# fulcrumgenomics/fgumi

Hardware: AMD Instinct MI355X
Metric: simplex consensus throughput, input raw reads/s (depth-8 x 150bp) (higher is better)
Workload: dtype f64

## Files before the change

fgumi_amd/csrc/api.cpp:

```cpp
#include <chrono>
#include <cstdio>
#include <stdexcept>
#include <cstring>
#include <mutex>
#include <map>
#include <mutex>
#include <string>
#include <thread>
#include "engine.h"
#include <gnu/libc-version.h>
#include <cmath>
#include "fastpath.h"
#include "host_common.h"
#include "simgen.h"
#include "canon_core.h"
#include "reject_core.h"
#include "aln_tags_core.h"

namespace fgx {
uint32_t launch_canon_molecules(hipStream_t s, bool codec, const canon::Params& P, const canon::CodecParams& PC, const uint8_t* d_blob,
                                const uint64_t* d_rec_off, const uint32_t* d_rec_len, const uint32_t* d_grp_first, const uint32_t* d_def, uint32_t nd,
                                const uint64_t* d_first, uint8_t* d_out, const uint64_t* d_out_off, uint32_t* d_out_len, int* d_status,
                                canon::Delta* d_delta, DevBuf& slabs);
void canon_layout_device(hipStream_t s, const uint32_t* d_rec_len, const uint32_t* d_grp_first, const uint32_t* d_def, uint32_t nd, unsigned long long* work,
// ... 1272 lines not shown
  double run = 0.0;
  for (uint32_t i = 0; i < n; i++) { run += (double)weights[i]; acc[i] = run; }
  const double total = acc[n - 1];
  for (uint32_t k = 1; k < world; k++) {
    const double want = total * (double)k / (double)world;
    const uint32_t idx = (uint32_t)(std::lower_bound(acc.begin(), acc.end(), want) - acc.begin());
    uint32_t c = idx + 1 > n ? n : idx + 1;
    if (c < cuts[k - 1]) c = cuts[k - 1];
    cuts[k] = c;
  }
  cuts[world] = n;
  for (uint32_t k = 1; k <= world; k++) if (cuts[k] < cuts[k - 1]) cuts[k] = cuts[k - 1];
  return 0;
}
uint32_t fgx_debug_last_split_chunks(const fgx_caller* c) { return (c && c->fast) ? c->fast->fp.last_split_chunks : 0u; }
uint32_t fgx_debug_last_big_families(const fgx_caller* c) { return (c && c->fast) ? c->fast->fp.last_big_families : 0u; }
uint32_t fgx_debug_last_meth_device(const fgx_caller* c) { return (c && c->fast) ? c->fast->fp.last_meth_device : 0u; }
uint32_t fgx_debug_last_deep_families(const fgx_caller* c) { return (c && c->fast) ? c->fast->fp.last_deep_families : 0u; }
void fgx_debug_last_split_builds(const fgx_caller* c, uint64_t* out4) {
  if (!out4) return;
  out4[0] = out4[1] = out4[2] = out4[3] = 0;
  if (c && c->fast) { const FastPath& f = c->fast->fp; out4[0] = f.last_packed_families; out4[1] = f.last_classic_families; out4[2] = f.last_split_build; out4[3] = f.last_first_stage_retries; }
}
void fgx_debug_last_chain(const fgx_caller* c, uint32_t* out2) { if (out2) { out2[0] = (c && c->fast) ? c->fast->fp.last_launches : 0u; out2[1] = (c && c->fast) ? c->fast->fp.last_host_syncs : 0u; } }
uint32_t fgx_debug_last_routed(const fgx_caller* c) { return (c && c->fast) ? c->fast->fp.last_routed : 0u; }
int fgx_debug_last_direct(const fgx_caller* c) { return (c && c->fast) ? c->fast->fp.last_direct : 0; }
void fgx_set_general_only(fgx_caller* c, int on) { if (c) c->general_only = on != 0; }
void fgx_set_fast_lds_bytes(fgx_caller* c, uint32_t bytes) { if (c) { if (!c->fast) c->fast = new FastState(); c->fast->fp.lds_tile_bytes_large = bytes; } }

int fgx_call_columns(fgx_caller* c, const uint8_t* bases, const uint8_t* quals, uint32_t n_cols, uint32_t depth, uint8_t* out_base,
                     uint8_t* out_qual, uint32_t* out_depth, uint32_t* out_errors) {
  if (!c) return 1;
  c->err.clear();
  try {
    ColumnBatch& B = c->batch;
    B.clear();
    std::vector<uint8_t> rb, rq;
    for (uint32_t j0 = 0; j0 < n_cols; j0 += 4096) {
      uint32_t w = std::min<uint32_t>(4096, n_cols - j0);
      uint32_t rd0 = (uint32_t)B.reads.size();
      for (uint32_t i = 0; i < depth; i++) {
        rb.resize(w); rq.resize(w);
        for (uint32_t k = 0; k < w; k++) { rb[k] = bases[(size_t)(j0 + k) * depth + i]; rq[k] = quals[(size_t)(j0 + k) * depth + i]; }
        B.add_read(rb.data(), rq.data(), w);
      }
      if (depth == 0) { B.add_job(rd0, 0, w); continue; }
// ... 129 lines not shown
```

fgumi_amd/csrc/fastpath.h:

```cpp
#pragma once
#include "engine.h"

namespace fgx {

constexpr int FAST_RX_CAP = 48;

struct EndDesc {
  uint64_t col_off;
  uint64_t first_off;
  uint64_t kept_off;
  uint32_t cons_len;
  uint32_t rec_size;
  uint16_t mi_off, cb_off;
  uint8_t mi_len, cb_len, rx_len, type;
  uint8_t has_cb, has_rx, valid, meth;
  char rx[FAST_RX_CAP];
};
struct MethSlot { uint32_t std_size, n_ml, mm_len, _pad; };

struct DuplexDesc {
  uint64_t a_off, b_off;
  uint32_t len;
  uint32_t first_rec;
  uint32_t cb_rec;
// ... 156 lines not shown
  const uint64_t* d_out_off;
  const uint64_t* d_slot_size;
  uint32_t n_slots;
  double ms_kernels, ms_k_family, ms_k_emit; uint64_t cols_used; uint64_t full_items;
};

struct FastPath {
  DevBuf d_ends, d_sizes, d_offsets, d_code, d_qual, d_depth, d_err, d_misc, d_deferred, d_out, d_scan_tmp, d_strings;
  uint32_t lds_tile_bytes = 12288;
  uint32_t lds_tile_bytes_large = 65536;
  DevBuf d_retry, d_bound, d_colbase, d_statslots, d_full_items, d_full_count, d_obs, d_retry2, d_retry_old;
  DevBuf d_w2img;
  DevBuf d_famdesc;
  DevBuf d_fwimg;
  DevBuf d_split_rec, d_split_fam, d_split_out, d_route, d_s2img;
  DevBuf d_big;
  uint32_t last_big_families = 0;
  uint32_t last_deep_families = 0;
  DevBuf d_deep_sizes, d_deep_row0, d_deep_rows, d_deep_fams, d_deep_out, d_deep_out2;
  DevBuf d_mflag, d_mu, d_mt, d_mslot, d_mcontigs;
  uint32_t last_meth_device = 0;
  uint32_t last_routed = 0;
  uint64_t last_packed_families = 0, last_classic_families = 0;
  uint32_t last_split_build = 0;
  uint32_t last_first_stage_retries = 0;
  uint32_t last_launches = 0, last_host_syncs = 0;
  DevBuf d_dir_size, d_dir_off, d_dir_base, d_slot_desc, d_slot_err, d_out2, d_scan_tmp2;
  bool direct_off = false;
  uint64_t dir_cap_min = 0;
  uint32_t dir_chunks_run = 0;
  int last_direct = 0;
  uint32_t lds_wave_bytes = 6144;
  uint32_t lds_wave_bytes_duplex = 8704;
  uint32_t lds_wave_bytes_codec = 5120;
  hipEvent_t ev[4] = {nullptr, nullptr, nullptr, nullptr};
  uint32_t pool_slack = 256; bool pool_init = false;
  uint32_t pool_div = 8;
  static constexpr int RUN_AGAIN_LARGER_POOL = -77;
  bool lds_attr_set = false, s2_attr_set = false, v2_attr_set = false;
  static constexpr int MAX_CHUNKS = 65;
  uint32_t last_split_chunks = 0;
  hipStream_t s2 = nullptr;
  hipEvent_t ev_chunk[MAX_CHUNKS] = {}, ev_cols[MAX_CHUNKS] = {}, ev_fin = nullptr, ev_sample = nullptr;
  int run(fgx_caller* c, const uint8_t* d_blob, uint64_t blob_len, const uint64_t* d_rec_off, const uint32_t* d_rec_len, uint32_t n_rec,
          const uint32_t* d_grp_first, uint32_t n_grp, FastResult* res);
  void release();
// ... 4 lines not shown
```

fgumi_amd/csrc/fastpath.hip:

```cpp
#if !defined(FGX_WAVEMU)
#include <hipcub/hipcub.hpp>
#endif
#include "bamrec.h"
#include "engine.h"
#include <cstdlib>
#include <memory>
#include <string>
#include <type_traits>
#include "fastpath.h"
#include "gate_core.h"
#include "packed_core.h"

#if defined(FGX_WAVEMU)
#define FGX_DYN_LDS(name) uint8_t* const name = wavemu::dyn_lds()
#define FGX_PIN(...) ((void)0)
#define FGX_UNDEF4(a, b, c, d) do { a = 0; b = 0; c = 0; d = 0; } while (0)
#define FGX_MEM_PIN() ((void)0)
#define FGX_CONST_AS
#else
#define FGX_DYN_LDS(name) extern __shared__ __align__(16) uint8_t name[]
#define FGX_PIN(...) asm volatile("" : __VA_ARGS__)
#define FGX_UNDEF4(a, b, c, d) asm volatile("" : "=v"(a), "=v"(b), "=v"(c), "=v"(d))
#define FGX_MEM_PIN() asm volatile("" ::: "memory")
#define FGX_CONST_AS __attribute__((address_space(4)))
// ... 3751 lines not shown
    hip_check(hipcub::DeviceScan::ExclusiveSum(fp.d_scan_tmp.p, tb, in, out, (int)n, s), what);
  }
  template <class Image> const void* table_image(DevBuf& d, void (*build)(Image&, const ConsensusTables&), const char* what) {
    if (!d.p) {
      const auto img = std::make_unique<Image>();
      build(*img, c->h_tables.t);
      d.reserve(sizeof(Image));
      hip_check(hipMemcpyAsync(d.p, img.get(), sizeof(Image), hipMemcpyHostToDevice, s), what);
      sync();
    }
    return d.p;
  }
  FastParams stage_params(uint32_t bytes, bool retry) {
    hip_check(hipMemsetAsync(cnt(MISC_N_RETRY), 0, 4, s), "memset");
    FastParams PS = P;
    PS.group_list = cur_list; PS.lds_wave_bytes = bytes;
    PS.retry = retry ? lists[out_list] : nullptr; PS.n_retry = cnt(MISC_N_RETRY);
    return PS;
  }
  void next_list(uint32_t n) { cur_list = lists[out_list]; n_cur = n; out_list ^= 1; }

  void set_up() {
    fp.last_meth_device = 0; fp.last_direct = 0; fp.last_split_chunks = 0;
    fp.last_routed = 0; fp.last_big_families = 0; fp.last_deep_families = 0; fp.last_packed_families = 0; fp.last_classic_families = 0; fp.last_split_build = 0; fp.last_first_stage_retries = 0;
    fp.d_ends.reserve((size_t)n_slots * (duplex ? sizeof(DuplexDesc) : codec ? sizeof(CodecDesc) : sizeof(EndDesc)));
    fp.d_sizes.reserve(((size_t)n_slots + 1) * 8);
    fp.d_offsets.reserve(((size_t)n_slots + 1) * 8);
    fp.d_deferred.reserve((size_t)n_grp * 4);
    fp.d_misc.reserve(MISC_WORDS * 8);
    hip_check(hipMemsetAsync(fp.d_misc.p, 0, MISC_WORDS * 8, s), "memset");
    misc = fp.d_misc.as<unsigned long long>();
    const std::string strs = c->prefix + c->rg;
    fp.d_strings.reserve(strs.size() + 16);
    if (!strs.empty()) hip_check(hipMemcpyAsync(fp.d_strings.p, strs.data(), strs.size(), hipMemcpyHostToDevice, s), "H2D strings");
    for (int i = 0; i < 4; i++) if (!fp.ev[i]) hip_check(hipEventCreate(&fp.ev[i]), "hipEventCreate");
    fp.d_bound.reserve(((size_t)n_grp + 1) * 8); fp.d_colbase.reserve(((size_t)n_grp + 1) * 8);
    fp.d_statslots.reserve((size_t)STAT_SLOTS * 32 * 8);
    hip_check(hipMemsetAsync(fp.d_statslots.p, 0, (size_t)STAT_SLOTS * 32 * 8, s), "memset");
    fp.d_famdesc.reserve((size_t)n_grp * 16);
    hip_check(hipEventRecord(c->ev0, s), "event");
    hip_check(hipEventRecord(fp.ev[0], s), "event");
    fpw = mean_recs >= 1.0 ? (uint32_t)(64.0 / mean_recs) : 16u;
    fpw = fpw < 1u ? 1u : fpw > 16u ? 16u : fpw;
    if (sw.split_fpw) fpw = sw.split_fpw;
    n_chunks = ps.chunks >= 1 ? (uint32_t)ps.chunks : std::min<uint32_t>(8u, std::max<uint32_t>(1u, n_grp / 150000u));
    if (n_chunks > (uint32_t)FastPath::MAX_CHUNKS - 1) n_chunks = FastPath::MAX_CHUNKS - 1;
    chunk_fam_raw = (n_grp + n_chunks - 1) / n_chunks;
// ... 502 lines not shown
    };
    read_counters();
    if ((duplex || codec) && (uint32_t)h_misc[MISC_N_SLOW] != 0) {
      if (codec) FGX_LAUNCH(k_emit_codec, wave_per_slot, dim3(256), 0, s, CE);
      else if (meth_dup) FGX_LAUNCH(HIP_KERNEL_NAME(k_emit_duplex<1>), wave_per_slot, dim3(256), 0, s, DE);
      else FGX_LAUNCH(HIP_KERNEL_NAME(k_emit_duplex<0>), wave_per_slot, dim3(256), 0, s, DE);
      read_counters();
    }
    float ms = 0, msf = 0, mse = 0;
    hip_check(hipEventElapsedTime(&ms, c->ev0, c->ev1), "elapsed");
    hip_check(hipEventElapsedTime(&msf, fp.ev[0], fp.ev[1]), "elapsed");
    hip_check(hipEventElapsedTime(&mse, fp.ev[2], fp.ev[3]), "elapsed");
    res->d_out = out_ptr;
    res->out_len = out_len;
    res->count = h_misc[MISC_STATS + 1];
    for (int i = 0; i < FGX_STATS_LEN; i++) res->stats[i] = h_misc[MISC_STATS + i];
    res->n_deferred = (uint32_t)(h_misc[MISC_N_DEFERRED] & 0xFFFFFFFFull);
    res->d_deferred = fp.d_deferred.as<uint32_t>();
    res->d_out_off = fp.d_offsets.as<uint64_t>();
    res->d_slot_size = fp.d_sizes.as<uint64_t>();
    res->n_slots = n_slots;
    res->ms_kernels = ms; res->ms_k_family = msf; res->ms_k_emit = mse;
    fp.last_packed_families = h_misc[MISC_BUILD_FAMILIES]; fp.last_classic_families = h_misc[MISC_BUILD_FAMILIES + 1];
    res->cols_used = h_misc[MISC_COLS_USED];
    res->full_items = n_full;
  }
};

int run_once(FastPath& fp, fgx_caller* c, const uint8_t* d_blob, uint64_t blob_len, const uint64_t* d_rec_off, const uint32_t* d_rec_len, uint32_t n_rec,
             const uint32_t* d_grp_first, uint32_t n_grp, FastResult* res) {
  memset(res, 0, sizeof(*res));
  fp.last_launches = 0; fp.last_host_syncs = 0;
  if (n_grp == 0) return 0;
  static const ProcessSwitches ps{};
  Batch b{fp, c, d_blob, blob_len, d_rec_off, d_rec_len, n_rec, d_grp_first, n_grp, res, ps};
  b.set_up();
  b.parse_first_chunk_early();
  b.bound_columns();
  b.fill_params();
  if (b.use_split) b.split_pipeline();
  if (b.simplex_v2) b.wave2_chain();
  b.family_wave_stages();
  b.deep_families();
  b.workgroup_families();
  if (const int rc = b.call_full()) return rc;
  if (b.direct) if (const int rc = b.check_direct()) return rc;
  b.place_records();
  b.write_records();
  return 0;
}

}

int FastPath::run(fgx_caller* c, const uint8_t* d_blob, uint64_t blob_len, const uint64_t* d_rec_off, const uint32_t* d_rec_len,
                  uint32_t n_rec, const uint32_t* d_grp_first, uint32_t n_grp, FastResult* res) {
  if (!pool_init) {
    if (const char* e = getenv("FGX_POOL_DIV")) { const long v = atol(e); if (v >= 1 && v <= (1 << 20)) pool_div = (uint32_t)v; }
    if (const char* e = getenv("FGX_POOL_SLACK")) { const long v = atol(e); if (v >= 1 && v <= 4096) pool_slack = (uint32_t)v; }
    pool_init = true;
  }
  for (;;) {
    const int rc = run_once(*this, c, d_blob, blob_len, d_rec_off, d_rec_len, n_rec, d_grp_first, n_grp, res);
    if (rc != RUN_AGAIN_LARGER_POOL) {
      if (const char* e = fgx_knob("FGX_S2_DEBUG")) if (atoi(e)) {
        uint32_t h[64];
        if (hipDeviceSynchronize() == hipSuccess && hipMemcpyFromSymbol(h, HIP_SYMBOL(g_s2_dbg), sizeof(h)) == hipSuccess) {
          fprintf(stderr, "[s2 packed] runs tried %u finished %u (columns for k_call_full %u) no room %u shape refused %u", h[0], h[1], h[2], h[3], h[42]);
          fprintf(stderr, "\n");
        }
      }
      return rc;
    }
  }
}

}

#if FGX_PHASE_TIMING
extern "C" int fgx_debug_phase_cycles(unsigned long long* out16, int reset) {
  unsigned long long h[64 * 16];
  if (hipMemcpyFromSymbol(h, HIP_SYMBOL(fgx::g_phase), sizeof(h)) != hipSuccess) return 1;
  for (int i = 0; i < 16; i++) { out16[i] = 0; for (int b = 0; b < 64; b++) out16[i] += h[b * 16 + i]; }
  if (reset) { memset(h, 0, sizeof(h)); if (hipMemcpyToSymbol(HIP_SYMBOL(fgx::g_phase), h, sizeof(h)) != hipSuccess) return 1; }
  return 0;
}
#endif
```

fgumi_amd/csrc/packed_core.h:

```cpp
#pragma once
#include <cstdint>
#include "consensus_math.h"

namespace fgx {
namespace pk {

constexpr uint32_t H = 0x80808080u;

FGX_HD uint32_t perm(uint32_t a, uint32_t b, uint32_t sel) {
#if defined(__HIP_DEVICE_COMPILE__)
  return __builtin_amdgcn_perm(a, b, sel);
#else
  const unsigned long long src = ((unsigned long long)a << 32) | b;
  uint32_t r = 0;
  for (int i = 0; i < 4; i++) {
    const uint32_t s = (sel >> (8 * i)) & 0xFFu;
    const uint32_t byte = s < 8u ? (uint32_t)(src >> (8 * s)) & 0xFFu : 0u;
    r |= byte << (8 * i);
  }
  return r;
#endif
}
FGX_HD uint32_t bitrev32(uint32_t x) {
#if defined(__HIP_DEVICE_COMPILE__)
// ... 79 lines not shown
    column_call(t, acc.s, acc.obs, &bi, &ql);
    if (bi == 0) t1[q] = ql;
  }
}

constexpr uint32_t T2_DIM = 94, T2_BYTES = T2_DIM * T2_DIM;
inline void fill_t2(uint8_t* t2 , const ConsensusTables& t) {
  for (uint32_t q1 = 0; q1 < T2_DIM; q1++)
    for (uint32_t q2 = 0; q2 < T2_DIM; q2++) {
      uint8_t& out = t2[q1 * T2_DIM + q2];
      out = 0xFF;
      ColumnAcc acc;
      acc.reset();
      acc.add(0, t.correct[q1], t.error_per_alt[q1]);
      acc.add(0, t.correct[q2], t.error_per_alt[q2]);
      if (!m_isfinite(acc.s[0]) || !m_isfinite(acc.s[1])) continue;
      int bi = -1;
      uint8_t ql = 0;
      column_call(t, acc.s, acc.obs, &bi, &ql);
      if (bi == 0) out = ql;
    }
}

}
}
```

fgumi_amd/csrc/simplex_split.inc:

```

#ifndef FGX_S2_OCC
#define FGX_S2_OCC 6
#endif
#ifndef FGX_S2_OCC_PACKED
#define FGX_S2_OCC_PACKED 7
#endif
#ifndef FGX_S2_PAIRS
#define FGX_S2_PAIRS 256
#endif

#ifndef FGX_S2_F32
#define FGX_S2_F32 1
#endif
#ifndef FGX_S2_FMASEL
#define FGX_S2_FMASEL 1
#endif
#ifndef FGX_S2_NOSUM
#define FGX_S2_NOSUM 1
#endif
#ifndef FGX_S2_PREGATE
#define FGX_S2_PREGATE 1
#endif
struct S2Lds {
  GateTables g;
// ... 468 lines not shown
__global__ __launch_bounds__(128) void k_split_parse(FastParams P, uint32_t g_begin, uint32_t n_grp, uint32_t fpw, uint64_t* __restrict__ bound, uint32_t max_ends,
                                                     uint4* __restrict__ fam_desc) {
  __shared__ __align__(16) uint8_t sTagCls[256];
  __shared__ __align__(16) uint8_t sWin[2 * SP_WAVE_LDS];
  fill_tag_classes(sTagCls);
  __syncthreads();
  const uint32_t wave = uni((blockIdx.x * blockDim.x + threadIdx.x) >> 6);
  const unsigned long long g0l = (unsigned long long)g_begin + (unsigned long long)wave * fpw;
  if (g0l >= n_grp) return;
  const uint32_t g0 = (uint32_t)g0l;
  const uint32_t nf = uni(n_grp - g0 < fpw ? n_grp - g0 : fpw);
  s2_parse_wave(P, g0, nf, sWin + (threadIdx.x >> 6) * SP_WAVE_LDS, sTagCls, bound, max_ends, fam_desc, [](uint32_t, uint32_t) {});
}

#if FGX_S2_PAIRS >= 256
#define S2_PAIR_OFF(q) ((q) << 4)
#else
#define S2_PAIR_OFF(q) (((q) < 93u ? (q) : 93u) << 4)
#endif
#ifndef FGX_S2_ABLATE
#define FGX_S2_ABLATE 0
#endif
#define S2_ABLATE_AFTER(k, sink) if (FGX_S2_ABLATE == (k)) { P.rec_sizes[slot0 + (lane & 1)] = (uint64_t)(sink); return; }
#ifndef FGX_S2_MIN_ITEMS
#define FGX_S2_MIN_ITEMS 8
#endif

#if FGX_S2_F32 && FGX_S2_FMASEL
#define S2_OBSERVE(q_, sb_, pr_) do { \
    const uint32_t w_q = (q_), w_c = ((uint32_t)(sb_) >> ish) & 15u; \
    const unsigned long long qm = __builtin_amdgcn_uicmp(w_q, min_bq, 35 ); \
    const unsigned long long bm = __builtin_amdgcn_uicmp(__builtin_amdgcn_ubfe(allow, w_c, 1u), 0u, 33 ); \
    suspect |= qm & ~bm; \
    const bool w_hit = __builtin_amdgcn_inverse_ballot_w64(qm & bm); \
    allow = w_hit ? 1u << w_c : allow; \
    const float w_sel = w_hit ? 1.0f : 0.0f; \
    const s2_f32x2 w_sel2 = {w_sel, w_sel}; \
    acc2 = __builtin_elementwise_fma((pr_), w_sel2, acc2);    \
    cntf += w_sel; \
  } while (0)
#else
#define S2_OBSERVE(q_, sb_, pr_) do { \
    const uint32_t w_q = (q_), w_c = ((uint32_t)(sb_) >> ish) & 15u; \
    const unsigned long long qm = __builtin_amdgcn_uicmp(w_q, min_bq, 35 ); \
    const unsigned long long bm = __builtin_amdgcn_uicmp(__builtin_amdgcn_ubfe(allow, w_c, 1u), 0u, 33 ); \
    suspect |= qm & ~bm; \
// ... 110 lines not shown
    if constexpr (TINY) {
      if (threadIdx.x < 24u) ((uint32_t*)&sL.t1[0])[threadIdx.x] = tiny_w;
      else if (threadIdx.x == 24u) sL.g.cap = tiny_w;
    } else {
      u32x4* const img_dst = (u32x4*)&sL;
#pragma unroll
      for (int u = 0; u < 6; u++) { const uint32_t ii = threadIdx.x + u * blockDim.x; if (ii < IMG_V) img_dst[ii] = im[u]; }
    }
  }
  const uint32_t body_off = d0.x, seq_rel = d0.y & 0xFFFF, l_seq = d0.y >> 16, clip = d0.z & 0xFFFF, ov_off1 = d0.z >> 16;
  const uint32_t ov_off2 = d0.w & 0xFFFF, ov_cnt = d0.w >> 16;
  const uint32_t slot = d1.x & 0xFF, mate_slot = (d1.x >> 8) & 0xFF, bits = (d1.x >> 16) & 0xFF, cb_len = d1.x >> 24;
  const uint32_t cb_rel = d1.y & 0xFFFF, mi_rel = d1.y >> 16, mi_len = d1.z & 0xFF, rx_rel = d1.z >> 16;
  const uint32_t ty = bits & 3u;
  const bool rev = (bits & 4u) != 0, has_cb = (bits & 8u) != 0;
  const unsigned long long lo_off = uniform_u64((unsigned long long)fd.x | ((unsigned long long)fd.y << 32));
  const uint8_t* const fbase = P.blob + lo_off;
  const uint32_t S0 = n * QS;
  if (act) *(uint2*)(W + ibase + 8u * slot) = make_uint2(body_off + seq_rel, l_seq);
  if constexpr (FUSED) wave_sync(); else __syncthreads();
  if (bail) return;
  {
    const uint32_t cpr = qc + sc, total = n * cpr;
    for (uint32_t t0 = 0; t0 < total; t0 += 256) {
      u32x4 v[4];
      uint32_t dst[4];
      bool on[4];
#pragma unroll
      for (int u = 0; u < 4; u++) {
        const uint32_t t = t0 + 64u * u + lane;
        const bool in = t < total;
        const uint32_t tt = in ? t : 0u;
        const uint32_t row = s2_mul24(tt, inv_cpr) >> 24;
        const uint32_t ch = tt - s2_mul24(row, cpr);
        const uint2 e = *(const uint2*)(W + ibase + 8u * row);
        const bool isq = ch < qc;
        const uint32_t c = isq ? ch : ch - qc;
        const uint32_t sbytes = (e.y + 1u) >> 1;
        const uint32_t src = e.x + (isq ? sbytes : 0u) + 16u * c;
        dst[u] = (isq ? row * QS : S0 + row * SS) + 16u * c;
        on[u] = in;
        const bool need_ld = in && 16u * c < (isq ? e.y : sbytes);
        u32x4 x = {0, 0, 0, 0};
        if (need_ld) __builtin_memcpy(&x, fbase + src, 16);
        v[u] = x;
      }
#pragma unroll
      for (int u = 0; u < 4; u++) if (on[u]) *(u32x4*)(W + dst[u]) = v[u];
    }
  }
  wave_sync();
  PH(1)
  const uint32_t my_q = slot * QS, my_s = S0 + slot * SS;
  if (__any(act && W[my_q] == 0xFF)) { to_route(); return; }
  S2_ABLATE_AFTER(1, W[my_s])

  const uint32_t min_bq = uni((uint32_t)P.min_input_bq & 0xFFu);
  uint32_t ov_agree = 0, ov_dis = 0, ov_corr = 0;
  {
    auto shared_base = [&](const bool in, const uint32_t o1, const uint32_t o2, const uint32_t q1, const uint32_t q2, const uint32_t sh1, const uint32_t sh2) {
      const uint32_t c1 = ((uint32_t)W[o1] >> sh1) & 15, c2 = ((uint32_t)W[o2] >> sh2) & 15;
      const uint32_t qa = W[q1], qb = W[q2];
      const bool valid = in && (c1 > c2 ? c1 : c2) != 15;
      const bool agree = c1 == c2;
      const uint32_t sm = qa + qb, nq = sm < 93 ? sm : 93;
      const int32_t d = (int32_t)qa - (int32_t)qb;
      const uint32_t ad = (uint32_t)(d < 0 ? -d : d), dq = ad < FGX_MIN_PHRED ? (uint32_t)FGX_MIN_PHRED : ad;
      const uint32_t cb = d == 0 ? 15u : d > 0 ? c1 : c2;
      const uint32_t newq = agree ? nq : dq;
      const bool drop = newq < min_bq;
      const uint32_t x1 = drop ? c1 : agree ? 0u : (c1 ^ cb), x2 = drop ? c2 : agree ? 0u : (c2 ^ cb);
      const bool changed = nq != qa || nq != qb;
      if (valid) {
        atomicXor((uint32_t*)(W + (o1 & ~3u)), x1 << (8 * (o1 & 3) + sh1));
        atomicXor((uint32_t*)(W + (o2 & ~3u)), x2 << (8 * (o2 & 3) + sh2));
        W[q1] = (uint8_t)newq; W[q2] = (uint8_t)newq;
      }
      const uint32_t na = (uint32_t)__popcll(__ballot(valid && agree)), nd = (uint32_t)__popcll(__ballot(valid && !agree));
      ov_agree += na; ov_dis += nd;
      ov_corr += (uint32_t)__popcll(__ballot(valid && agree && changed)) + 2u * nd;
    };
    const unsigned long long om = __ballot(act && ov_cnt != 0);
    if (om) {
      const uint32_t np = (uint32_t)__popcll(om), fp = (uint32_t)__builtin_ctzll(om);
      const uint32_t cn0 = rlane(ov_cnt, fp);
      if (ov_uniform && np > 1u && cn0 < 64u) {
        const uint32_t oo1 = rlane(ov_off1, fp), oo2 = rlane(ov_off2, fp);
        if (act && ov_cnt != 0) *(uint16_t*)(W + ibase + 2u * (uint32_t)__popcll(om & below)) = (uint16_t)(slot | (mate_slot << 8));
        wave_sync();
        const uint32_t inv = uni((uint32_t)(1048576.0f / (float)cn0) + 2u);
        const uint32_t total = np * cn0;
        for (uint32_t t0 = 0; t0 < total; t0 += 64) {
          const uint32_t t = t0 + lane;
          const bool in = t < total;
          const uint32_t tt = in ? t : 0u;
          const uint32_t pk = s2_mul24(tt, inv) >> 20, w = tt - s2_mul24(pk, cn0);
          const uint32_t rows = *(const uint16_t*)(W + ibase + 2u * pk), r1 = rows & 0xFF, r2 = rows >> 8;
          const uint32_t i1 = oo1 + w, i2 = oo2 + w;
          shared_base(in, S0 + r1 * SS + (i1 >> 1), S0 + r2 * SS + (i2 >> 1), r1 * QS + i1, r2 * QS + i2, (~i1 & 1) << 2, (~i2 & 1) << 2);
        }
      } else {
        const uint32_t mt_q = mate_slot * QS, mt_s = S0 + mate_slot * SS;
        const uint32_t my_q0 = slot * QS, my_s0 = S0 + slot * SS;
        for (unsigned long long pm = om; pm; pm &= pm - 1) {
          const uint32_t a = (uint32_t)__builtin_ctzll(pm);
          const uint32_t sa = rlane(my_s0, a), qa0 = rlane(my_q0, a), sb = rlane(mt_s, a), qb0 = rlane(mt_q, a);
          const uint32_t cn = rlane(ov_cnt, a);
          const uint32_t i1 = rlane(ov_off1, a) + lane, i2 = rlane(ov_off2, a) + lane;
          uint32_t o1 = sa + (i1 >> 1), o2 = sb + (i2 >> 1), q1 = qa0 + i1, q2 = qb0 + i2;
          const uint32_t sh1 = (~i1 & 1) << 2, sh2 = (~i2 & 1) << 2;
          for (uint32_t w0 = 0; w0 < cn; w0 += 64, o1 += 32, o2 += 32, q1 += 64, q2 += 64) shared_base(w0 + lane < cn, o1, o2, q1, q2, sh1, sh2);
        }
      }
    }
  }
  const uint32_t ov_bases = ov_agree + ov_dis;
  wave_sync();
  PH(3)
  S2_ABLATE_AFTER(3, ov_bases + ov_corr + W[my_s])

  const uint32_t fl = l_seq > clip ? l_seq - clip : 0u;
  if (act) {
    uint32_t z0, z1;
    if (!rev) { z0 = fl; z1 = ty == 2u ? len_b : len_a; } else { z0 = 0; z1 = clip < l_seq ? clip : l_seq; }
// ... 343 lines not shown
  bool ires_asked = false;
  auto run_cols_packed = [&](const uint32_t cnt_a, const uint32_t cnt_b, const uint32_t m, const bool last_run) -> bool {
    const uint32_t nsafe = P.s2_nsafe;
    const uint32_t ga = cnt_a ? (len_a + 7u) >> 3 : 0u, gb = cnt_b ? (len_b + 7u) >> 3 : 0u;
    const bool dbg = (P.s2_packed & 2u) != 0;
    if (!(P.s2_packed && m >= nsafe && m <= S2_PACKED_MAX_ROWS && P.min_reads <= nsafe && min_bq <= 128u && ((QS & 7u) | (SS & 3u)) == 0u && ga + gb <= 64u &&
          S0 + s2_mul24(n, SS) < 65536u && lc_a + lc_b < 65536u)) {
      if (dbg && lane == 0) atomicAdd(&g_s2_dbg[42], 1u);
      return false;
    }
    if (dbg && lane == 0) atomicAdd(&g_s2_dbg[0], 1u);
    const bool in_b = lane >= ga, inl = lane < ga + gb;
    const uint32_t k = inl ? (in_b ? lane - ga : lane) : 0u;
    const bool lrev = (in_b ? rev_b : rev_a) != 0;
    const uint32_t lenE = in_b ? len_b : len_a, cntE = in_b ? cnt_b : cnt_a;
    const uint32_t rowE = in_b ? m_a : 0u;
    const uint32_t qaddr0 = s2_mul24(rowE, QS) + 8u * k, saddr0 = S0 + s2_mul24(rowE, SS) + 4u * k;
    const uint32_t H = pk::H;
    uint32_t nfl, nfh;
    pk::count_masks(lenE, k, &nfl, &nfh);
    const uint32_t mb4 = min_bq * 0x01010101u;
    pk::Acc A;
    pk::acc_reset(A);
    {
      uint32_t qj = qaddr0, sj = saddr0, j = 0;
      for (; j + 4 <= m; j += 4, qj += 4 * QS, sj += 4 * SS) {
        const uint2 q0 = *(const uint2*)(W + qj), q1 = *(const uint2*)(W + qj + QS), q2 = *(const uint2*)(W + qj + 2 * QS), q3 = *(const uint2*)(W + qj + 3 * QS);
        const uint32_t b0 = *(const uint32_t*)(W + sj), b1_ = *(const uint32_t*)(W + sj + SS), b2_ = *(const uint32_t*)(W + sj + 2 * SS), b3_ = *(const uint32_t*)(W + sj + 3 * SS);
        pk::acc_row(A, q0.x, q0.y, b0, mb4, nfl, nfh); pk::acc_row(A, q1.x, q1.y, b1_, mb4, nfl, nfh);
        pk::acc_row(A, q2.x, q2.y, b2_, mb4, nfl, nfh); pk::acc_row(A, q3.x, q3.y, b3_, mb4, nfl, nfh);
      }
      for (; j < m; j++, qj += QS, sj += SS) { const uint2 q0 = *(const uint2*)(W + qj); const uint32_t b0 = *(const uint32_t*)(W + sj); pk::acc_row(A, q0.x, q0.y, b0, mb4, nfl, nfh); }
    }
    PH(9)
    pk::Out F;
    pk::finalize(A, inl, lrev, lenE, cntE, k, nsafe, sT.cap, P.min_cons_bq, P.min_reads, F);
    const int32_t c_lo = F.c_lo, lo_s = F.lo_s, hi_s = F.hi_s;
    const uint32_t* const code2 = F.code2; const uint32_t* const qual2 = F.qual2; const uint32_t* const dep4 = F.dep4;
    const uint32_t* const flag2 = F.flag2; const uint32_t* const full2 = F.valid2;
    PH(10)
    uint32_t fm = (flag2[0] >> 7) | (flag2[1] >> 3);
    const uint32_t fc = (uint32_t)__builtin_popcount(fm);
    const unsigned long long pb0 = __ballot((fc & 1u) != 0), pb1 = __ballot((fc & 2u) != 0), pb2 = __ballot((fc & 4u) != 0), pb3 = __ballot((fc & 8u) != 0);
    const uint32_t T = uni((uint32_t)__popcll(pb0) + 2u * (uint32_t)__popcll(pb1) + 4u * (uint32_t)__popcll(pb2) + 8u * (uint32_t)__popcll(pb3));
    const uint32_t oc0 = (in_b ? offB : offA) + (uint32_t)c_lo;
    const uint32_t list = (P.lds_wave_bytes - 8u * T) & ~7u;
// ... 91 lines not shown
    } else {
      if (ne >= 1u && surv_a == 1u) single_end(mem_a, lc_a, offA);
      if (ne == 2u && surv_b == 1u) single_end(mem_b, lc_b, offB);
    }
    const bool both = multi_a && multi_b && m_a == m_b;
    const uint32_t nruns = both ? 1u : (multi_a ? 1u : 0u) + (multi_b ? 1u : 0u);
#pragma unroll 1
    for (uint32_t ri = 0; ri < nruns && !gone; ri++) {
      const bool first_is_a = both || multi_a;
      const bool run_a = ri == 0 && first_is_a, run_b = both || !run_a;
      const uint32_t rc_a = run_a ? lc_a : 0u, rc_b = run_b ? lc_b : 0u, rc_m = run_a ? m_a : m_b;
      if constexpr (COLS == 1) { if (!run_cols_packed(rc_a, rc_b, rc_m, ri + 1 == nruns)) gone = true; }
      else run_cols(rc_a, rc_b, rc_m);
    }
    if (gone) { if (gone_far) to_route(); else to_retry(); return; }
  }
  PH(6)
  S2_ABLATE_AFTER(6, icnt + rej + ov_bases + ov_corr)

  uint32_t ires = 0;
  if (ires_asked) ires = ires_early;
  else if (icnt && lane == 0) ires = atomicAdd(&P.full_count[my_list], icnt);
  {
    leave(COLS == 1 ? 0x81u : 1u, (ne << 8) | (type_a << 16) | (fk_a << 24), fk_b | (surv_a << 8) | (surv_b << 16) | (n << 24), lc_a | (lc_b << 16), rej, ov_agree, ov_dis);
    if (lane == 0) ((uint32_t*)&P.split_out[g])[6] = ov_corr;
  }
  if constexpr (DIRECT != 0) {
    uint32_t mx = acc_max, mn = acc_min, sm = acc_sum;
    for (int o = 32; o > 0; o >>= 1) { mx = s2_pkmax(mx, (uint32_t)__shfl_xor((int)mx, o)); mn = s2_pkmin(mn, (uint32_t)__shfl_xor((int)mn, o)); sm += (uint32_t)__shfl_xor((int)sm, o); }
    mx = uni(mx); mn = uni(mn); sm = uni(sm);
    auto tail = [&](const S2DirRec& R, uint32_t sumd) {
      if (lane == 0) {
        SlotDesc sd; sd.out_off = dir_off_early + R.base; sd.lc_seq = R.Lc | (R.o_seq << 16); sd.sum_depth = sumd;
        P.slot_desc[slot0 + R.type] = sd;
      }
    };
    if (ne >= 1u) tail(RA, sm & 0xFFFFu);
    if (ne == 2u) tail(RB, sm >> 16);
    if (lane == 0) ((uint32_t*)&P.split_out[g])[7] = (mx & 0xFFu) | ((mn & 0xFFu) << 8) | (((mx >> 16) & 0xFFu) << 16) | (((mn >> 16) & 0xFFu) << 24);
    dir_tables(type_a == 0u ? RA.size : 0u, type_a == 0u ? 0u : RA.size, RB.size);
  }
  if (icnt) {
    wave_sync();
    uint32_t base = uni(ires), l = my_list, done = 0, tries = 0;
    bool overflow = false;
    if (multi_items) {
      for (;;) {
// ... 63 lines not shown
  constexpr uint32_t IMG_V = TINY ? 0u : (uint32_t)((FGX_S2_F32 ? S2_HEAD_BYTES : (uint32_t)sizeof(S2Lds)) / 16);
  static_assert(IMG_V <= 6 * 64 || !FGX_S2_F32, "table image larger than six loads per thread");
  const u32x4* const img_src = (const u32x4*)P.s2_image;
  u32x4 im[6];
  uint32_t tiny_w = 0;
  if constexpr (TINY) {
    static_assert(offsetof(S2Lds, t1) % 4 == 0 && offsetof(GateTables, cap) % 4 == 0, "the packed build copies its tables as 32-bit words");
    const uint32_t* const w = (const uint32_t*)P.s2_image;
    if (threadIdx.x < 24u) tiny_w = w[offsetof(S2Lds, t1) / 4 + threadIdx.x];
    else if (threadIdx.x == 24u) tiny_w = w[(offsetof(S2Lds, g) + offsetof(GateTables, cap)) / 4];
  } else {
#pragma unroll
    for (int u = 0; u < 6; u++) { const uint32_t ii = threadIdx.x + u * blockDim.x; im[u] = img_src[ii < IMG_V ? ii : 0u]; }
  }
  uint8_t* W = dyn + (size_t)wv * P.lds_wave_bytes;
  const uint32_t my_list = blockIdx.x & (N_LISTS - 1);
  s2_cols_family<QS_T, SS_T, DIRECT, COLS, false>(P, g, bail, tiny_w, im, W, sL, lane, my_list);
}

__global__ __launch_bounds__(256) void k_split_finish(FastParams P, uint32_t count) {
  typedef uint32_t u32x4 __attribute__((ext_vector_type(4)));
  const uint32_t gi = blockIdx.x * blockDim.x + threadIdx.x;
  const uint32_t lane = threadIdx.x & 63;
  uint32_t c_total = 0, c_cons = 0, c_insuf = 0, c_zero = 0, c_orphan = 0, c_agree = 0, c_dis = 0, c_corr = 0, c_packed = 0, c_classic = 0;
  if (gi < count) {
    const uint32_t g = P.group_list ? P.group_list[gi] : P.g0 + gi;
    const SplitOut O = P.split_out[g];
    const uint32_t slot0 = 3 * g;
    const uint32_t o_status = O.status & 0x7Fu;
    const bool padded = (O.status & 0x80u) != 0;
    if (o_status == 2) { c_total = O.n; c_insuf = O.n; }
    const bool direct = P.out != nullptr;
    if (o_status != 0 && !direct) {
      EndDesc* D = &P.ends[slot0];
      D[0].valid = 0; D[1].valid = 0; D[2].valid = 0;
      P.rec_sizes[slot0] = 0; P.rec_sizes[slot0 + 1] = 0; P.rec_sizes[slot0 + 2] = 0;
    }
    if (o_status == 1) {
      c_packed = padded ? 1u : 0u; c_classic = padded ? 0u : 1u;
      c_total = O.n; c_cons = O.ne;
      c_insuf = O.rej & 0xFF; c_zero = (O.rej >> 8) & 0xFF; c_orphan = O.rej >> 16;
      c_agree = O.ov_agree; c_dis = O.ov_dis; c_corr = O.ov_corr;
      const uint4 fd = P.fam_desc[g];
      const unsigned long long lo_off = (unsigned long long)fd.x | ((unsigned long long)fd.y << 32);
      const uint32_t r0 = P.grp_first[g];
      const SplitFam F = P.split_fam[g];
      const SplitRec R0 = P.split_rec[r0];
      const uint64_t col_base = P.col_base[g];
      if (direct) {
        const uint8_t* const fbase = P.blob + lo_off;
        const uint8_t* const strs = (const uint8_t*)P.strings;
        const uint32_t mi0 = R0.mi_len, nm = P.prefix_len + 1u + mi0;
        const uint8_t* const mi_src = fbase + R0.mi_rel;
        uint64_t rec_off = P.dir_off[g];
        for (uint32_t k = 0; k < O.ne; k++) {
          const uint32_t Lc = k == 0 ? O.lc_a : O.lc_b, e_type = k == 0 ? O.type_a : 2u;
          const uint32_t fk = k == 0 ? O.fk_a : O.fk_b, kept = k == 0 ? O.kept_a : O.kept_b;
          const uint32_t dst = k == 0 ? O.depth_stats & 0xFFFFu : O.depth_stats >> 16, maxd = dst & 0xFFu, mind = dst >> 8;
          const SplitRec RK = P.split_rec[r0 + fk];
          const bool hcb = P.cell0 && (RK.bits & 8u);
          const uint32_t cbl = RK.cb_len, rxn = F.rx_all ? kept : 0u, rxl = F.rx_len;
          const uint32_t o_seq = 36u + nm + 1u, o_rg = o_seq + ((Lc + 1u) >> 1) + Lc, o_t3 = o_rg + 3u + P.rg_len + 1u;
          const uint32_t o_cd = o_t3 + 15u + 8u, o_ce = o_cd + 2u * Lc + 8u, o_mi = P.per_base_tags ? o_ce + 2u * Lc : o_t3 + 15u;
          const uint32_t o_cb = o_mi + 3u + mi0 + 1u, o_rx = o_cb + (hcb ? 3u + cbl + 1u : 0u), size = o_rx + (rxn ? 3u + rxl + 1u : 0u);
// ... 66 lines not shown
              const uint32_t ch = (v >> (8 * bb)) & 0xFF, up = ch & 0xDFu, idx = up - 'A';
              const bool dna = idx < 26 && ((0x00082045u >> idx) & 1u);
              const uint32_t o = (4 * w + bb < rx_ulen) ? ((rx_cnt > 1 && dna) ? up : ch) : 0u;
              out |= o << (8 * bb);
            }
          }
          rxw[w] = out;
        }
        const uint64_t col_off = col_base + (padded ? (k == 0 ? S2_PAD_FRONT : s2_padded_b(O.lc_a)) : (k == 0 ? 0u : (uint32_t)O.lc_a)), kept_off = lo_off + RK.body_off;
        const u32x4 p0 = {(uint32_t)col_off, (uint32_t)(col_off >> 32), (uint32_t)lo_off, (uint32_t)(lo_off >> 32)};
        const u32x4 p1 = {(uint32_t)kept_off, (uint32_t)(kept_off >> 32), Lc, size};
        const u32x4 p2 = {(uint32_t)R0.mi_rel | ((uint32_t)RK.cb_rel << 16), mi0_len | (cbl << 8) | (rx_ulen << 16) | (e_type << 24),
                          (hcb ? 1u : 0u) | ((rx_cnt ? 1u : 0u) << 8) | (1u << 16), rxw[0]};
        const u32x4 p3 = {rxw[1], rxw[2], rxw[3], rxw[4]}, p4 = {rxw[5], rxw[6], rxw[7], rxw[8]}, p5 = {rxw[9], rxw[10], rxw[11], 0u};
        u32x4* dst = (u32x4*)&P.ends[slot0 + e_type];
        dst[0] = p0; dst[1] = p1; dst[2] = p2; dst[3] = p3; dst[4] = p4; dst[5] = p5;
        P.rec_sizes[slot0 + e_type] = (uint64_t)size + 4;
      }
    }
  }
  const uint32_t t_cons = wave_sum(c_cons), t_total = wave_sum(c_total), t_insuf = wave_sum(c_insuf), t_zero = wave_sum(c_zero), t_orphan = wave_sum(c_orphan);
  const uint32_t t_agree = wave_sum(c_agree), t_dis = wave_sum(c_dis), t_corr = wave_sum(c_corr);
  const uint32_t t_packed = wave_sum(c_packed), t_classic = wave_sum(c_classic);
  if (lane == 0) {
    unsigned long long* st = P.stats + (size_t)((blockIdx.x * 4 + (threadIdx.x >> 6)) & (STAT_SLOTS - 1)) * 32;
    if (t_total) atomicAdd(&st[0], (unsigned long long)t_total);
    if (t_cons) atomicAdd(&st[1], (unsigned long long)t_cons);
    const uint32_t filt = t_insuf + t_zero + t_orphan;
    if (filt) atomicAdd(&st[2], (unsigned long long)filt);
    if (t_insuf) atomicAdd(&st[3 + FGX_REJ_INSUFFICIENT_READS], (unsigned long long)t_insuf);
    if (t_zero) atomicAdd(&st[3 + FGX_REJ_ZERO_LENGTH_AFTER_TRIMMING], (unsigned long long)t_zero);
    if (t_orphan) atomicAdd(&st[3 + FGX_REJ_ORPHAN_CONSENSUS], (unsigned long long)t_orphan);
    if (t_agree + t_dis) atomicAdd(&st[24], (unsigned long long)(t_agree + t_dis));
    if (t_agree) atomicAdd(&st[25], (unsigned long long)t_agree);
    if (t_dis) atomicAdd(&st[26], (unsigned long long)t_dis);
    if (t_corr) atomicAdd(&st[27], (unsigned long long)t_corr);
    if (t_packed) atomicAdd(&st[28], (unsigned long long)t_packed);
    if (t_classic) atomicAdd(&st[29], (unsigned long long)t_classic);
  }
}
```

Before: 2.899 billion.

## Pack overlap correction into 8-column SWAR lanes and stage narrow rows per 16 lanes

Adds a packed overlap path in which each lane processes eight overlapping columns at once. It does this with SWAR byte and nibble arithmetic and only falls back to a per-slot scalar loop for disagreeing columns, writing changes back with atomic XORs. It also adds a row-staging loop for families whose rows fit in 16 chunks, so four rows are copied per lane per pass instead of a flat 256-item loop. New counters record which overlap form each family took. The aim is fewer per-column iterations in the overlap and staging phases, at the cost of more complex bit logic and LDS atomics.

```diff
diff --git a/fgumi_amd/csrc/api.cpp b/fgumi_amd/csrc/api.cpp
--- a/fgumi_amd/csrc/api.cpp
+++ b/fgumi_amd/csrc/api.cpp
@@ -1318,6 +1318,11 @@
   out4[0] = out4[1] = out4[2] = out4[3] = 0;
   if (c && c->fast) { const FastPath& f = c->fast->fp; out4[0] = f.last_packed_families; out4[1] = f.last_classic_families; out4[2] = f.last_split_build; out4[3] = f.last_first_stage_retries; }
 }
+void fgx_debug_last_overlap_forms(const fgx_caller* c, uint64_t* out2) {
+  if (!out2) return;
+  out2[0] = out2[1] = 0;
+  if (c && c->fast) { out2[0] = c->fast->fp.last_ov_packed_families; out2[1] = c->fast->fp.last_ov_base_families; }
+}
 void fgx_debug_last_chain(const fgx_caller* c, uint32_t* out2) { if (out2) { out2[0] = (c && c->fast) ? c->fast->fp.last_launches : 0u; out2[1] = (c && c->fast) ? c->fast->fp.last_host_syncs : 0u; } }
 uint32_t fgx_debug_last_routed(const fgx_caller* c) { return (c && c->fast) ? c->fast->fp.last_routed : 0u; }
 int fgx_debug_last_direct(const fgx_caller* c) { return (c && c->fast) ? c->fast->fp.last_direct : 0; }
diff --git a/fgumi_amd/csrc/fastpath.h b/fgumi_amd/csrc/fastpath.h
--- a/fgumi_amd/csrc/fastpath.h
+++ b/fgumi_amd/csrc/fastpath.h
@@ -202,6 +202,7 @@
   uint32_t last_meth_device = 0;
   uint32_t last_routed = 0;
   uint64_t last_packed_families = 0, last_classic_families = 0;
+  uint64_t last_ov_packed_families = 0, last_ov_base_families = 0;
   uint32_t last_split_build = 0;
   uint32_t last_first_stage_retries = 0;
   uint32_t last_launches = 0, last_host_syncs = 0;
diff --git a/fgumi_amd/csrc/fastpath.hip b/fgumi_amd/csrc/fastpath.hip
--- a/fgumi_amd/csrc/fastpath.hip
+++ b/fgumi_amd/csrc/fastpath.hip
@@ -3797,7 +3797,7 @@
 
   void set_up() {
     fp.last_meth_device = 0; fp.last_direct = 0; fp.last_split_chunks = 0;
-    fp.last_routed = 0; fp.last_big_families = 0; fp.last_deep_families = 0; fp.last_packed_families = 0; fp.last_classic_families = 0; fp.last_split_build = 0; fp.last_first_stage_retries = 0;
+    fp.last_routed = 0; fp.last_big_families = 0; fp.last_deep_families = 0; fp.last_packed_families = 0; fp.last_classic_families = 0; fp.last_ov_packed_families = 0; fp.last_ov_base_families = 0; fp.last_split_build = 0; fp.last_first_stage_retries = 0;
     fp.d_ends.reserve((size_t)n_slots * (duplex ? sizeof(DuplexDesc) : codec ? sizeof(CodecDesc) : sizeof(EndDesc)));
     fp.d_sizes.reserve(((size_t)n_slots + 1) * 8);
     fp.d_offsets.reserve(((size_t)n_slots + 1) * 8);
@@ -4346,6 +4346,7 @@
     res->n_slots = n_slots;
     res->ms_kernels = ms; res->ms_k_family = msf; res->ms_k_emit = mse;
     fp.last_packed_families = h_misc[MISC_BUILD_FAMILIES]; fp.last_classic_families = h_misc[MISC_BUILD_FAMILIES + 1];
+    fp.last_ov_packed_families = h_misc[MISC_BUILD_FAMILIES + 2]; fp.last_ov_base_families = h_misc[MISC_BUILD_FAMILIES + 3];
     res->cols_used = h_misc[MISC_COLS_USED];
     res->full_items = n_full;
   }
@@ -4390,6 +4391,7 @@
         uint32_t h[64];
         if (hipDeviceSynchronize() == hipSuccess && hipMemcpyFromSymbol(h, HIP_SYMBOL(g_s2_dbg), sizeof(h)) == hipSuccess) {
           fprintf(stderr, "[s2 packed] runs tried %u finished %u (columns for k_call_full %u) no room %u shape refused %u", h[0], h[1], h[2], h[3], h[42]);
+          fprintf(stderr, "; row loop: %u rows, floor branch taken in %u", h[4], h[5]);
           fprintf(stderr, "\n");
         }
       }
diff --git a/fgumi_amd/csrc/packed_core.h b/fgumi_amd/csrc/packed_core.h
--- a/fgumi_amd/csrc/packed_core.h
+++ b/fgumi_amd/csrc/packed_core.h
@@ -125,5 +125,66 @@
     }
 }
 
+struct OvOut { uint32_t xq1l, xq1h, xq2l, xq2h, xc1, xc2, agree, dis, corr; };
+FGX_HD uint32_t nibswap(uint32_t w) { return ((w >> 4) & 0x0F0F0F0Fu) | ((w & 0x0F0F0F0Fu) << 4); }
+FGX_HD uint32_t popc32(uint32_t x) {
+#if defined(__HIP_DEVICE_COMPILE__)
+  return (uint32_t)__popc(x);
+#else
+  return (uint32_t)__builtin_popcount(x);
+#endif
+}
+FGX_HD void overlap_slot(uint32_t wa, uint32_t wb, uint32_t c1w, uint32_t c2w, uint32_t s, uint32_t floor, OvOut& o) {
+  const uint32_t sh8 = 8u * (s & 3u), sh4 = 4u * s;
+  const uint32_t qa = (wa >> sh8) & 0xFFu, qb = (wb >> sh8) & 0xFFu, c1 = (c1w >> sh4) & 15u, c2 = (c2w >> sh4) & 15u;
+  const bool agree = c1 == c2;
+  const uint32_t sm = qa + qb, nq = sm < 93u ? sm : 93u;
+  const uint32_t ad = qa > qb ? qa - qb : qb - qa, dq = ad < (uint32_t)FGX_MIN_PHRED ? (uint32_t)FGX_MIN_PHRED : ad;
+  const uint32_t cb = qa == qb ? 15u : qa > qb ? c1 : c2;
+  const uint32_t newq = agree ? nq : dq;
+  const bool drop = newq < floor;
+  const uint32_t x1 = drop ? c1 : agree ? 0u : (c1 ^ cb), x2 = drop ? c2 : agree ? 0u : (c2 ^ cb);
+  const uint32_t xa = (qa ^ newq) << sh8, xb = (qb ^ newq) << sh8;
+  const bool low = s < 4u;
+  o.xq1l |= low ? xa : 0u; o.xq1h |= low ? 0u : xa; o.xq2l |= low ? xb : 0u; o.xq2h |= low ? 0u : xb;
+  o.xc1 |= x1 << sh4; o.xc2 |= x2 << sh4;
+  const bool changed = nq != qa || nq != qb;
+  o.agree += agree ? 1u : 0u; o.dis += agree ? 0u : 1u; o.corr += agree ? (changed ? 1u : 0u) : 2u;
+}
+FGX_HD uint32_t overlap_half(uint32_t fl, uint32_t a, uint32_t b, uint32_t F4, uint32_t* xa_out, uint32_t* xb_out, OvOut& o) {
+  uint32_t t = fl & 0xFFFFu;
+  t = (t | (t << 8)) & 0x00FF00FFu; t = (t | (t << 4)) & 0x0F0F0F0Fu;
+  const uint32_t vB = (t << 7) & H, neB = (t << 6) & H;
+  const uint32_t s = (a & 0x7F7F7F7Fu) + (b & 0x7F7F7F7Fu);
+  const uint32_t ge = (((s & 0x7F7F7F7Fu) + 0x22222222u) | s) & H;
+  const uint32_t gM = (ge << 1) - (ge >> 7);
+  const uint32_t nq = (s & ~gM) | (0x5D5D5D5Du & gM);
+  const uint32_t geF = ((nq | H) - F4) & H;
+  const uint32_t fast = vB & ~neB & ~(a | b) & geF;
+  const uint32_t fM = (fast << 1) - (fast >> 7);
+  const uint32_t xa = (a ^ nq) & fM, xb = (b ^ nq) & fM;
+  const uint32_t ch = xa | xb;
+  const uint32_t nz = (((ch & 0x7F7F7F7Fu) + 0x7F7F7F7Fu) | ch) & H;
+  *xa_out = xa; *xb_out = xb;
+  o.agree += popc32(fast); o.corr += popc32(nz);
+  return vB & ~fast;
+}
+FGX_HD void overlap8(uint32_t q1l, uint32_t q1h, uint32_t q2l, uint32_t q2h, uint32_t c1, uint32_t c2, uint32_t lo, uint32_t hi, uint32_t floor, OvOut& o) {
+  const uint32_t hiM = hi >= 8u ? 0xFFFFFFFFu : (1u << (4u * hi)) - 1u, loM = lo >= 8u ? 0u : 0xFFFFFFFFu << (4u * lo);
+  uint32_t t1 = c1 & (c1 >> 1), t2 = c2 & (c2 >> 1);
+  t1 &= t1 >> 2; t2 &= t2 >> 2;
+  const uint32_t d = c1 ^ c2;
+  const uint32_t ne = ((((d & 0x77777777u) + 0x77777777u) | d) >> 3) & 0x11111111u;
+  const uint32_t valid = 0x11111111u & hiM & loM & ~(t1 | t2);
+  const uint32_t fl = valid | (ne << 1);
+  const uint32_t F4 = (floor < 94u ? floor : 94u) * 0x01010101u;
+  o.xc1 = 0; o.xc2 = 0; o.agree = 0; o.dis = 0; o.corr = 0;
+  const uint32_t slow_l = overlap_half(fl, q1l, q2l, F4, &o.xq1l, &o.xq2l, o), slow_h = overlap_half(fl >> 16, q1h, q2h, F4, &o.xq1h, &o.xq2h, o);
+  for (uint32_t m = (slow_l >> 7) | (slow_h >> 3); m; m &= m - 1u) {
+    const uint32_t bit = (uint32_t)__builtin_ctz(m), s = (bit >> 3) + (bit & 4u);
+    overlap_slot(s < 4u ? q1l : q1h, s < 4u ? q2l : q2h, c1, c2, s, floor, o);
+  }
+}
+
 }
 }
diff --git a/fgumi_amd/csrc/simplex_split.inc b/fgumi_amd/csrc/simplex_split.inc
--- a/fgumi_amd/csrc/simplex_split.inc
+++ b/fgumi_amd/csrc/simplex_split.inc
@@ -514,6 +514,12 @@
 #define FGX_S2_ABLATE 0
 #endif
 #define S2_ABLATE_AFTER(k, sink) if (FGX_S2_ABLATE == (k)) { P.rec_sizes[slot0 + (lane & 1)] = (uint64_t)(sink); return; }
+#ifndef FGX_S2_OVPACK
+#define FGX_S2_OVPACK 1
+#endif
+#ifndef FGX_S2_STAGE16
+#define FGX_S2_STAGE16 1
+#endif
 #ifndef FGX_S2_MIN_ITEMS
 #define FGX_S2_MIN_ITEMS 8
 #endif
@@ -670,6 +676,38 @@
   if (bail) return;
   {
     const uint32_t cpr = qc + sc, total = n * cpr;
+#if FGX_S2_STAGE16
+    if (cpr <= 16u) {
+      const uint32_t ch = lane & 15u;
+      const bool isq = ch < qc;
+      const uint32_t rl = ch < cpr ? lane >> 4 : 64u;
+      const uint32_t qsel = isq ? ~0u : 0u;
+      const uint32_t c16 = 16u * (isq ? ch : ch - qc);
+      const uint32_t cend = isq ? c16 : 2u * c16;
+      const uint32_t dcol = (isq ? 0u : S0) + c16, dstride = isq ? QS : SS;
+      const uint32_t nlast = n - 1u;
+      for (uint32_t rb = 0; rb < n; rb += 16) {
+        uint2 e[4];
+        u32x4 v[4];
+        uint32_t row[4];
+#pragma unroll
+        for (int u = 0; u < 4; u++) {
+          row[u] = rb + 4u * u + rl;
+          e[u] = *(const uint2*)(W + ibase + 8u * (row[u] < nlast ? row[u] : nlast));
+        }
+#pragma unroll
+        for (int u = 0; u < 4; u++) {
+          const bool need_ld = (row[u] < n) & (cend < e[u].y);
+          u32x4 x = {0, 0, 0, 0};
+          if (need_ld) __builtin_memcpy(&x, fbase + (e[u].x + (((e[u].y + 1u) >> 1) & qsel) + c16), 16);
+          v[u] = x;
+        }
+        const uint32_t dst0 = s2_mul24(row[0], dstride) + dcol;
+#pragma unroll
+        for (int u = 0; u < 4; u++) if (row[u] < n) *(u32x4*)(W + dst0 + 4u * u * dstride) = v[u];
+      }
+    } else
+#endif
     for (uint32_t t0 = 0; t0 < total; t0 += 256) {
       u32x4 v[4];
       uint32_t dst[4];
@@ -705,6 +743,7 @@
 
   const uint32_t min_bq = uni((uint32_t)P.min_input_bq & 0xFFu);
   uint32_t ov_agree = 0, ov_dis = 0, ov_corr = 0;
+  uint32_t ov_form = 0;
   {
     auto shared_base = [&](const bool in, const uint32_t o1, const uint32_t o2, const uint32_t q1, const uint32_t q2, const uint32_t sh1, const uint32_t sh2) {
       const uint32_t c1 = ((uint32_t)W[o1] >> sh1) & 15, c2 = ((uint32_t)W[o2] >> sh2) & 15;
@@ -736,8 +775,54 @@
         const uint32_t oo1 = rlane(ov_off1, fp), oo2 = rlane(ov_off2, fp);
         if (act && ov_cnt != 0) *(uint16_t*)(W + ibase + 2u * (uint32_t)__popcll(om & below)) = (uint16_t)(slot | (mate_slot << 8));
         wave_sync();
+        const uint32_t total = np * cn0;
+#if FGX_S2_OVPACK
+        if (COLS == 1 && total > 64u) {
+          ov_form |= 1u;
+          const uint32_t g0 = oo1 >> 3, end1 = oo1 + cn0, nI = ((end1 + 7u) >> 3) - g0;
+          const uint32_t invI = uni((uint32_t)(1048576.0f / (float)nI) + 2u);
+          const uint32_t totI = np * nI, delta = oo2 - oo1;
+          uint32_t l_agree = 0, l_dis = 0, l_corr = 0;
+          for (uint32_t t0 = 0; t0 < totI; t0 += 64) {
+            const uint32_t t = t0 + lane;
+            const bool in = t < totI;
+            const uint32_t tt = in ? t : 0u;
+            const uint32_t pi = s2_mul24(tt, invI) >> 20, j = tt - s2_mul24(pi, nI);
+            const uint32_t rows = *(const uint16_t*)(W + ibase + 2u * pi), r1 = rows & 0xFF, r2 = rows >> 8;
+            const uint32_t g = g0 + j, left = end1 - 8u * g;
+            const uint32_t lo = j == 0u ? (oo1 & 7u) : 0u, hi = !in ? 0u : left < 8u ? left : 8u;
+            const uint32_t qa1 = r1 * QS + 8u * g, ca1 = S0 + r1 * SS + 4u * g;
+            const int32_t b2 = (int32_t)(8u * g + delta), a2 = b2 >> 3;
+            const uint32_t sh = (uint32_t)b2 & 7u, a2c = a2 < 0 ? 0u : (uint32_t)a2, a2n = (uint32_t)(a2 + 1);
+            const uint32_t qrow2 = r2 * QS, crow2 = S0 + r2 * SS;
+            const uint2 Q1 = *(const uint2*)(W + qa1), QA = *(const uint2*)(W + qrow2 + 8u * a2c), QB = *(const uint2*)(W + qrow2 + 8u * a2n);
+            const uint32_t C1 = *(const uint32_t*)(W + ca1), CA = *(const uint32_t*)(W + crow2 + 4u * a2c), CB = *(const uint32_t*)(W + crow2 + 4u * a2n);
+            const uint64_t qlo = (uint64_t)QA.x | ((uint64_t)QA.y << 32), qhi = (uint64_t)QB.x | ((uint64_t)QB.y << 32);
+            const uint64_t q2w = sh ? (qlo >> (8u * sh)) | (qhi << (64u - 8u * sh)) : qlo;
+            const uint32_t c2 = (uint32_t)((((uint64_t)pk::nibswap(CB) << 32) | pk::nibswap(CA)) >> (4u * sh));
+            pk::OvOut o;
+            pk::overlap8(Q1.x, Q1.y, (uint32_t)q2w, (uint32_t)(q2w >> 32), pk::nibswap(C1), c2, lo, hi, min_bq, o);
+            l_agree += o.agree; l_dis += o.dis; l_corr += o.corr;
+            if (o.xq1l) atomicXor((uint32_t*)(W + qa1), o.xq1l);
+            if (o.xq1h) atomicXor((uint32_t*)(W + (qa1 + 4u)), o.xq1h);
+            if (o.xc1) atomicXor((uint32_t*)(W + ca1), pk::nibswap(o.xc1));
+            const uint64_t x2 = (uint64_t)o.xq2l | ((uint64_t)o.xq2h << 32);
+            const uint64_t x2l = x2 << (8u * sh), x2h = sh ? x2 >> (64u - 8u * sh) : 0ull;
+            const uint32_t qb2 = qrow2 + 8u * (uint32_t)a2, cb2 = crow2 + 4u * (uint32_t)a2;
+            if ((uint32_t)x2l) atomicXor((uint32_t*)(W + qb2), (uint32_t)x2l);
+            if ((uint32_t)(x2l >> 32)) atomicXor((uint32_t*)(W + (qb2 + 4u)), (uint32_t)(x2l >> 32));
+            if ((uint32_t)x2h) atomicXor((uint32_t*)(W + (qb2 + 8u)), (uint32_t)x2h);
+            if ((uint32_t)(x2h >> 32)) atomicXor((uint32_t*)(W + (qb2 + 12u)), (uint32_t)(x2h >> 32));
+            const uint64_t y2 = (uint64_t)o.xc2 << (4u * sh);
+            if ((uint32_t)y2) atomicXor((uint32_t*)(W + cb2), pk::nibswap((uint32_t)y2));
+            if ((uint32_t)(y2 >> 32)) atomicXor((uint32_t*)(W + (cb2 + 4u)), pk::nibswap((uint32_t)(y2 >> 32)));
+          }
+          ov_agree = wave_sum(l_agree); ov_dis = wave_sum(l_dis); ov_corr = wave_sum(l_corr);
+        } else
+#endif
+        {
+        ov_form |= 2u;
         const uint32_t inv = uni((uint32_t)(1048576.0f / (float)cn0) + 2u);
-        const uint32_t total = np * cn0;
         for (uint32_t t0 = 0; t0 < total; t0 += 64) {
           const uint32_t t = t0 + lane;
           const bool in = t < total;
@@ -747,7 +832,9 @@
           const uint32_t i1 = oo1 + w, i2 = oo2 + w;
           shared_base(in, S0 + r1 * SS + (i1 >> 1), S0 + r2 * SS + (i2 >> 1), r1 * QS + i1, r2 * QS + i2, (~i1 & 1) << 2, (~i2 & 1) << 2);
         }
+        }
       } else {
+        ov_form |= 2u;
         const uint32_t mt_q = mate_slot * QS, mt_s = S0 + mate_slot * SS;
         const uint32_t my_q0 = slot * QS, my_s0 = S0 + slot * SS;
         for (unsigned long long pm = om; pm; pm &= pm - 1) {
@@ -1137,6 +1224,13 @@
     const uint32_t mb4 = min_bq * 0x01010101u;
     pk::Acc A;
     pk::acc_reset(A);
+#if FGX_KNOBS
+    if (dbg) {
+      uint32_t taken = 0, qj = qaddr0;
+      for (uint32_t j = 0; j < m; j++, qj += QS) { const uint2 q0 = *(const uint2*)(W + qj); taken += __any(pk::any_below(q0.x, q0.y, mb4, nfl, nfh)) ? 1u : 0u; }
+      if (lane == 0) { atomicAdd(&g_s2_dbg[4], m); atomicAdd(&g_s2_dbg[5], taken); }
+    }
+#endif
     {
       uint32_t qj = qaddr0, sj = saddr0, j = 0;
       for (; j + 4 <= m; j += 4, qj += 4 * QS, sj += 4 * SS) {
@@ -1274,7 +1368,7 @@
   if (ires_asked) ires = ires_early;
   else if (icnt && lane == 0) ires = atomicAdd(&P.full_count[my_list], icnt);
   {
-    leave(COLS == 1 ? 0x81u : 1u, (ne << 8) | (type_a << 16) | (fk_a << 24), fk_b | (surv_a << 8) | (surv_b << 16) | (n << 24), lc_a | (lc_b << 16), rej, ov_agree, ov_dis);
+    leave(COLS == 1 ? 0x81u : 1u, (ne << 8) | (type_a << 16) | (fk_a << 24), fk_b | (surv_a << 8) | (surv_b << 16) | (n << 24), lc_a | (lc_b << 16), rej | (ov_form << 24), ov_agree, ov_dis);
     if (lane == 0) ((uint32_t*)&P.split_out[g])[6] = ov_corr;
   }
   if constexpr (DIRECT != 0) {
@@ -1384,7 +1478,7 @@
   typedef uint32_t u32x4 __attribute__((ext_vector_type(4)));
   const uint32_t gi = blockIdx.x * blockDim.x + threadIdx.x;
   const uint32_t lane = threadIdx.x & 63;
-  uint32_t c_total = 0, c_cons = 0, c_insuf = 0, c_zero = 0, c_orphan = 0, c_agree = 0, c_dis = 0, c_corr = 0, c_packed = 0, c_classic = 0;
+  uint32_t c_total = 0, c_cons = 0, c_insuf = 0, c_zero = 0, c_orphan = 0, c_agree = 0, c_dis = 0, c_corr = 0, c_packed = 0, c_classic = 0, c_ovpack = 0, c_ovbase = 0;
   if (gi < count) {
     const uint32_t g = P.group_list ? P.group_list[gi] : P.g0 + gi;
     const SplitOut O = P.split_out[g];
@@ -1401,7 +1495,8 @@
     if (o_status == 1) {
       c_packed = padded ? 1u : 0u; c_classic = padded ? 0u : 1u;
       c_total = O.n; c_cons = O.ne;
-      c_insuf = O.rej & 0xFF; c_zero = (O.rej >> 8) & 0xFF; c_orphan = O.rej >> 16;
+      c_insuf = O.rej & 0xFF; c_zero = (O.rej >> 8) & 0xFF; c_orphan = (O.rej >> 16) & 0xFF;
+      c_ovpack = (O.rej >> 24) & 1u; c_ovbase = (O.rej >> 25) & 1u;
       c_agree = O.ov_agree; c_dis = O.ov_dis; c_corr = O.ov_corr;
       const uint4 fd = P.fam_desc[g];
       const unsigned long long lo_off = (unsigned long long)fd.x | ((unsigned long long)fd.y << 32);
@@ -1514,6 +1609,7 @@
   const uint32_t t_cons = wave_sum(c_cons), t_total = wave_sum(c_total), t_insuf = wave_sum(c_insuf), t_zero = wave_sum(c_zero), t_orphan = wave_sum(c_orphan);
   const uint32_t t_agree = wave_sum(c_agree), t_dis = wave_sum(c_dis), t_corr = wave_sum(c_corr);
   const uint32_t t_packed = wave_sum(c_packed), t_classic = wave_sum(c_classic);
+  const uint32_t t_ovpack = wave_sum(c_ovpack), t_ovbase = wave_sum(c_ovbase);
   if (lane == 0) {
     unsigned long long* st = P.stats + (size_t)((blockIdx.x * 4 + (threadIdx.x >> 6)) & (STAT_SLOTS - 1)) * 32;
     if (t_total) atomicAdd(&st[0], (unsigned long long)t_total);
@@ -1529,5 +1625,7 @@
     if (t_corr) atomicAdd(&st[27], (unsigned long long)t_corr);
     if (t_packed) atomicAdd(&st[28], (unsigned long long)t_packed);
     if (t_classic) atomicAdd(&st[29], (unsigned long long)t_classic);
+    if (t_ovpack) atomicAdd(&st[30], (unsigned long long)t_ovpack);
+    if (t_ovbase) atomicAdd(&st[31], (unsigned long long)t_ovbase);
   }
 }
```

Result: no change. 2.876 billion (median of 2 runs) (-0.8%).
